# DAGroup-PKU/MHLA

Measured on AMD Instinct MI355X. Metric: MHLA fwd+bwd tokens/sec at (B,N,H,D), higher is better.
Workload: dtype bf16; 1 GPU; block-mix MHLA op fwd+bwd, per GPU B=8 N=4096 H=16 D=64 M=64 S=64 bf16 (BASELINE.json configs[1]); global_batch=8, parallelism=dp1 (batch shards, dW all-reduce only)

## Files before the change

mhla_amd/csrc/capi.hip:

```cpp
#include "capi_common.hpp"
#include "fused.hpp"
#include "fused_tile16.hpp"
#include "smalln.hpp"
#include "smalln_f32.hpp"

using namespace mhla;
using namespace mhla::capi;

namespace mhla {
namespace capi {
extern template int bm_fwd_typed<float, false>(const BmCall&);
extern template int bm_fwd_typed<bf16_t, true>(const BmCall&);
extern template int bm_fwd_typed<bf16_t, false>(const BmCall&);
extern template int bm_fwd_typed<f16_t, false>(const BmCall&);
extern template int bm_bwd_typed<float, false>(const BmCall&);
extern template int bm_bwd_typed<bf16_t, true>(const BmCall&);
extern template int bm_bwd_typed<bf16_t, false>(const BmCall&);
extern template int bm_bwd_typed<f16_t, false>(const BmCall&);
}
}

namespace {

template <int MODE>
// ... 129 lines not shown
}

extern "C" {


int mhla_abi_version(void) { return MHLA_ABI_VERSION; }

#ifndef MHLA_BUILD_FLAGS
#define MHLA_BUILD_FLAGS "unknown"
#endif
const char* mhla_build_flags(void) { return MHLA_BUILD_FLAGS; }

void mhla_prof_enable(int on) {
    std::lock_guard<std::mutex> lk(g_prof_mu);
    g_prof_on = on != 0;
}

int mhla_prof_report(char* buf, size_t cap) {
    std::vector<ProfRec> recs;
    {
        std::lock_guard<std::mutex> lk(g_prof_mu);
        recs.swap(g_prof);
    }
    std::map<std::string, std::pair<long, double>> agg;
    for (auto& r : recs) {
        float ms = 0.f;
        (void)hipEventSynchronize(r.e1);
        (void)hipEventElapsedTime(&ms, r.e0, r.e1);
        auto& a = agg[r.name];
        a.first += 1;
        a.second += ms;
        (void)hipEventDestroy(r.e0);
        (void)hipEventDestroy(r.e1);
    }
    std::string out;
    char line[256];
    for (auto& kv : agg) {
        snprintf(line, sizeof(line), "%s %ld %.6f\n", kv.first.c_str(), kv.second.first, kv.second.second);
        out += line;
    }
    if (!buf || cap == 0) return (int)out.size();
    const size_t n = out.size() < cap - 1 ? out.size() : cap - 1;
    memcpy(buf, out.data(), n);
    buf[n] = 0;
    return (int)n;
}
const char* mhla_last_error(void) { return g_err; }

int mhla_set_option(const char* name, int value) {
    if (name && !strcmp(name, "bwd_two_launches")) return g_two_launches.exchange(value != 0);
    if (name && !strcmp(name, "debug_drop_signal")) return g_drop_signal.exchange(value != 0);
    if (name && !strcmp(name, "fp32_summaries")) return g_no_p24.exchange(value != 0);
    if (name && !strcmp(name, "recut_kernels")) return g_recut.exchange(value != 0);
    return fail(MHLA_EINVAL, "mhla_set_option: unknown option '%s'", name ? name : "(null)");
}

void mhla_debug_set_trace(void* buf) { g_trace = (unsigned long long*)buf; }

int mhla_blockmix_fwd_keeps_state(int B, int H, int M, int S, int D, int dtype, int split, unsigned flags) {
    (void)B; (void)H;
    switch (bm_route(M, S, D, dtype, split != 0, flags)) {
        case BM_SNF: case BM_SN: return 0;
        case BM_FAST: return 1;
        default: return sp_shape_ok(D, flags) ? 1 : 0;
    }
}

size_t mhla_blockmix_fwd_ws_bytes(int B, int H, int M, int S, int D, int dtype, int split, unsigned flags) {
    const size_t gen = bm_carve_for(nullptr, B, H, M, S, D, dtype, flags, true).total_fwd;
    return bm_fast_layout(M, S, D, dtype, split != 0, flags) ? std::max(gen, fast_carve(nullptr, B, H, M, S).total_fwd) : gen;
}
size_t mhla_blockmix_bwd_ws_bytes(int B, int H, int M, int S, int D, int dtype, int split, unsigned flags) {
    return bwd_ws_body_bytes(B, H, M, S, D, dtype, split, flags) + 16;
}

static BmCall bm_call(mhla_view q_num, mhla_view k_num, mhla_view v, mhla_view q_den, mhla_view k_den, const float* W, int ldw, const int32_t* block_index,
                      int B, int H, int M, int S, int D, int dtype, float eps, unsigned flags, void* stream, const float* rcos, const float* rsin, long ldr) {
    BmCall c{};
    c.normalize = q_den.ptr != nullptr;
    c.split = c.normalize && (q_den.ptr != q_num.ptr || k_den.ptr != k_num.ptr);
    c.q_num = q_num; c.k_num = k_num; c.v = v; c.q_den = c.normalize ? q_den : q_num; c.k_den = c.normalize ? k_den : k_num;
    c.W = W; c.ldw = ldw; c.block_index = block_index; c.B = B; c.H = H; c.M = M; c.S = S; c.D = D; c.dtype = dtype; c.eps = eps; c.flags = flags;
    c.st = (hipStream_t)stream; c.rcos = rcos; c.rsin = rsin; c.ldr = ldr;
    return c;
}
static int bm_typed(const BmCall& c, const bool FWD) {
    switch (c.dtype) {
        case MHLA_F32: return FWD ? bm_fwd_typed<float, false>(c) : bm_bwd_typed<float, false>(c);
        case MHLA_BF16:
            if (bm_sum16(c.D, c.dtype, c.flags)) return FWD ? bm_fwd_typed<bf16_t, true>(c) : bm_bwd_typed<bf16_t, true>(c);
            return FWD ? bm_fwd_typed<bf16_t, false>(c) : bm_bwd_typed<bf16_t, false>(c);
        case MHLA_F16: return FWD ? bm_fwd_typed<f16_t, false>(c) : bm_bwd_typed<f16_t, false>(c);
        default: return fail(MHLA_EINVAL, "unknown dtype %d", c.dtype);
    }
}

static fast::SnArgs sn_args(const BmCall& c, void* dwp) {
    fast::SnArgs sa{};
    sa.q = cv(c.q_num); sa.k = cv(c.k_num); sa.v = cv(c.v); sa.idx = c.block_index; sa.W = c.W; sa.ldw = c.ldw;
    sa.H = c.H; sa.M = c.M; sa.D = c.D; sa.eps = c.eps; sa.relu = c.relu(); sa.normalize = c.normalize;
    if (!dwp) { sa.out = cmv(c.out); return sa; }
    sa.o = c.normalize ? cv(c.outv) : cv(c.q_num); sa.dout = cv(c.dout); sa.dq = cmv(c.dq_num); sa.dk = cmv(c.dk_num); sa.dv = cmv(c.dv); sa.dwp = (float*)dwp;
    return sa;
}
static int sn_fwd(const BmCall& c, BmRoute r) {
    const fast::SnArgs sa = sn_args(c, nullptr);
// ... 277 lines not shown
```

mhla_amd/csrc/capi_bm_typed.hpp:

```cpp
#pragma once
#include "capi_common.hpp"
#include "blockmix.hpp"
#include "split.hpp"
#include "split16.hpp"
#include "mixh2.hpp"

namespace mhla {
namespace capi {

static_assert(sp::mixr_te<4, SF_BF16>() == mixr_slice(true) && sp::mixr_te<4, SF_F32>() == mixr_slice(false) && sp::mixr_te<4, SF_P24>() == mixr_slice(false), "bm_plan's resident-mixing rule");
template <int DT> constexpr int sp_state_threads() {
#ifdef MHLA_SP_STATE_4WAVES
    return NTHREADS;
#else
    return DT == 8 ? 512 : NTHREADS;
#endif
}
#ifndef SP_MIXH2_IH
#define SP_MIXH2_IH 2
#endif
#ifndef SP_MIXH2_RT
#define SP_MIXH2_RT 1
#endif

// ... 109 lines not shown
    constexpr bool PACKED = bm_fmt_built<ET, DT, S16, SF_P24>();
    const MixOp o = mix_op(p, c, TRANS);
    const bool wz = c.normalize && p.wz_fused;
    const char* name = p.n_mix[TRANS];
    const MixArgs tiled{o.W, o.ldw, o.in, o.out, o.M, o.E, o.es}, dense{o.W, o.ldw, o.in, o.out, o.M, o.E, TRANS ? 0 : o.es};
    switch (p.mix[TRANS]) {
        case K_MIX:
            return launch(k_mix<TRANS, 0>, dim3((unsigned)((o.E + MIX_TE - 1) / MIX_TE), (o.M + MIX_TI - 1) / MIX_TI, o.BH), dim3(NTHREADS), MIX_SMEM_FLOATS * 4, o.st, name, dense);
        case K_SP_MIX:
            if (p.fmt == PLAIN) return launch(sp::k_sp_mix<TRANS, PLAIN>, dim3((unsigned)((o.E + sp::SPM_TE - 1) / sp::SPM_TE), (o.M + 63) / 64, o.BH), dim3(NTHREADS), sp::sp_mix_smem<PLAIN>(), o.st, name, tiled);
            break;
        case K_SP_MIXR_DMA:
            if constexpr (S16) return sp_mixr_dma<TRANS>(o, wz, name);
            break;
        case K_SP_MIXR:
            if (TRANS == 1 && p.dw_fused) {
                if constexpr (TRANS == 1) {
                    if (p.fmt == SF_P24) { if constexpr (PACKED) return sp_mixr<1, SF_P24, true>(o, p.nw, wz, name, parts); }
                    else if (p.fmt == SF_F32) return sp_mixr<1, SF_F32, true>(o, p.nw, wz, name, parts);
                }
            } else if (p.fmt == SF_P24) { if constexpr (PACKED) return sp_mixr<TRANS, SF_P24, false>(o, p.nw, wz, name); }
            else if (p.fmt == PLAIN) return sp_mixr<TRANS, PLAIN, false>(o, p.nw, wz, name);
            break;
        case K_SP_MIXH: case K_SP_MIXH2:
            if constexpr (PACKED) return sp_mixh<TRANS>(o, p.mix[TRANS], p.nw, TRANS && p.dw_fused, wz, name, parts);
            break;
        default: break;
    }
    return not_built<ET, DT>(name, p.fmt);
}
template <int TRANS>
int launch_wz(const float* W, int ldw, const float* x, float* out, int BH, int M, int S, float eps, hipStream_t st) {
    return launch(k_wz<TRANS>, dim3((S + 63) / 64, (M + 63) / 64, BH), dim3(NTHREADS), 0, st, N_WZ[TRANS], W, ldw, x, out, M, S, eps);
}

template <typename ET, int DT, int TRANS, bool S16>
int bm_state(const BmPlan& p, const BmCall& c, const StateArgs& a) {
    constexpr bool F32 = std::is_same<ET, float>::value;
    constexpr int SNT = sp_state_threads<DT>();
    const dim3 g(c.M, c.B * c.H);
    const char* name = p.n_state[TRANS];
    if (p.state == K_BM_STATE) return launch(k_bm_state<ET, DT, TRANS>, g, dim3(NTHREADS), state_smem_floats<DT>() * 4, c.st, name, a);
    if (p.state == K_S16_STATE) return launch(s16::k_s16_state<TRANS>, dim3((c.M + s16::WPB - 1) / s16::WPB, c.B * c.H), dim3(64 * s16::WPB), s16::state_smem(), c.st, name, a);
    if (p.rope) {
        constexpr sp::StateVar ROPE{.rope = true};
        if (p.fmt == SF_P24) {
            if constexpr (F32 && bm_fmt_built<ET, DT, S16, SF_P24>()) return launch(sp::k_sp_state<ET, DT, TRANS, SNT, SF_P24, ROPE>, g, dim3(SNT), sp::sp_state_smem<DT>(), c.st, name, a);
        } else if (p.fmt == sf_plain<S16>()) {
            if constexpr (F32 || TRANS == 0) return launch(sp::k_sp_state<ET, DT, TRANS, SNT, sf_plain<S16>(), ROPE>, g, dim3(SNT), sp::sp_state_smem<DT>(), c.st, name, a);
        }
        return not_built<ET, DT>(name, p.fmt);
    }
    if constexpr (TRANS == 0 && bm_fmt_built<ET, DT, S16, SF_H16>()) {
        if (p.fmt == SF_H16 && !(c.normalize && c.split) && g_recut.load())
            return launch(sp::k_sp_state<ET, DT, 0, SNT, SF_H16, sp::StateVar{.ts = false}>, g, dim3(SNT), sp::sp_state_smem<DT>(), c.st, name, a);
    }
    return with_fmt<ET, DT, S16>(p.fmt, name, [&]<int FMT>() {
        constexpr int smem = (sf_packed(FMT) && TRANS && sizeof(ET) == 2 && DT <= 4) ? sp::sp_state_rd_smem<DT, sp::sp_payrd<ET, DT, FMT>()>() : sp::sp_state_smem<DT>();
        return launch(sp::k_sp_state<ET, DT, TRANS, SNT, FMT>, g, dim3(SNT), smem, c.st, name, a);
    });
}
template <typename ET, int DT, bool S16>
int bm_state_and_mix(const BmPlan& p, const BmCall& c) {
    const BmWs& w = c.w;
    StateArgs a{};
    a.rcos = c.rcos; a.rsin = c.rsin; a.ldr = c.ldr;
    a.x = cv(c.k_num); a.y = cv(c.v); a.kd = cv(c.k_den); a.qd = cv(c.q_den); a.idx = c.block_index;
    a.out = w.kv; a.ksum = w.ksum; a.zo = w.z; a.es = w.es;
    a.H = c.H; a.M = c.M; a.S = c.S; a.D = c.D; a.eps = c.eps; a.relu = c.relu(); a.normalize = c.normalize; a.split = c.split;
    RC((bm_state<ET, DT, 0, S16>(p, c, a)));
    RC((bm_mix<ET, DT, 0, S16>(p, c)));
    if (p.wz_kernel) RC(launch_wz<0>(c.W, c.ldw, w.z, w.ninv, c.B * c.H, c.M, c.S, c.eps, c.st));
    return MHLA_OK;
}

template <typename ET, int DT, bool S16, typename TO = ET, bool EPI = false>
int sp_out(const BmPlan& p, const BmCall& c, const OutArgs& o, const char* name) {
    const dim3 g(c.M, c.B * c.H), blk(sp::SP_OUT_T);
    if constexpr (!EPI && bm_fmt_built<ET, DT, S16, SF_H16>() && DT <= 4) {
        if (p.fmt == SF_H16 && bm_one_tile(c.S))
            return launch(sp::k_sp_out<ET, DT, TO, SF_H16, sp::OutVar{.one = true}>, g, blk, sp::sp_out_smem<DT, SF_H16>(), c.st, name, o);
    }
    return with_fmt<ET, DT, S16>(p.fmt, name, [&]<int FMT>() {
        return launch(sp::k_sp_out<ET, DT, TO, FMT, sp::OutVar{.epi = EPI}>, g, blk, sp::sp_out_smem<DT, FMT>(), c.st, name, o);
    });
}
inline OutArgs out_args(const BmCall& c) {
    OutArgs o{};
    o.rcos = c.rcos; o.rsin = c.rsin; o.ldr = c.ldr;
    o.q = cv(c.q_num); o.idx = c.block_index; o.W = c.W; o.ldw = c.ldw; o.g = c.w.g; o.ninv = c.w.ninv;
    o.H = c.H; o.M = c.M; o.S = c.S; o.D = c.D; o.eps = c.eps; o.es = c.w.es; o.relu = c.relu(); o.normalize = c.normalize;
    return o;
}
template <typename ET, int DT, bool S16>
int bm_out(const BmPlan& p, const BmCall& c, OutArgs& o, const char* name) {
    if (p.out == K_BM_OUT) return launch(k_bm_out<ET, DT>, dim3(c.M, c.B * c.H), dim3(NTHREADS), out_smem_floats<DT>() * 4, c.st, name, o);
    if (p.out == K_S16_OUT) return launch(s16::k_s16_out<0>, dim3((c.M + s16::WPB - 1) / s16::WPB, c.B * c.H), dim3(64 * s16::WPB), s16::out_smem(), c.st, name, o);
    if (!c.epi) return sp_out<ET, DT, S16>(p, c, o, name);
    if constexpr (std::is_same<ET, float>::value) {
        o.nw = c.nw; o.neps = c.neps; o.gate = cv(c.gate);
        if (c.out_dtype == MHLA_BF16) return sp_out<float, DT, S16, bf16_t, true>(p, c, o, name);
        if (c.out_dtype == MHLA_F16) return sp_out<float, DT, S16, f16_t, true>(p, c, o, name);
        return sp_out<float, DT, S16, float, true>(p, c, o, name);
    }
    return not_built<ET, DT>(name, p.fmt);
}

inline int sp_dwr_splits(int BH, long E) {
    int ns = (256 + BH - 1) / BH;
    if (ns > DW_MAX_SPLIT) ns = DW_MAX_SPLIT;
    while (ns > 1 && E / ns < 256) --ns;
// ... 149 lines not shown
```

mhla_amd/csrc/capi_common.hpp:

```cpp
#pragma once
#include "../../include/mhla_hip.h"

#include <algorithm>
#include <atomic>
#include <cstdarg>
#include <cstdio>
#include <cstdlib>
#include <cstring>
#include <map>
#include <mutex>
#include <string>
#include <vector>

#include "common.hpp"

namespace mhla {
namespace capi {


inline thread_local char g_err[512] = "";

inline int fail(int code, const char* fmt, ...) {
    va_list ap;
    va_start(ap, fmt);
// ... 9 lines not shown
inline std::atomic<bool> g_prof_on{false};
inline std::vector<ProfRec> g_prof;

template <typename K>
int launch(K kernel, dim3 grid, dim3 block, size_t smem, hipStream_t stream, const char* name, auto... args) {
    if (smem > 48 * 1024) {
        static std::mutex mu;
        static std::map<std::pair<const void*, int>, size_t> done;
        int dev = 0;
        (void)hipGetDevice(&dev);
        const std::pair<const void*, int> key(reinterpret_cast<const void*>(kernel), dev);
        std::lock_guard<std::mutex> lk(mu);
        auto it = done.find(key);
        if (it == done.end() || it->second < smem) {
            hipError_t e = hipFuncSetAttribute(key.first, hipFuncAttributeMaxDynamicSharedMemorySize, (int)smem);
            if (e != hipSuccess) return fail(MHLA_ELAUNCH, "%s: hipFuncSetAttribute(%zu B LDS): %s", name, smem, hipGetErrorString(e));
            done[key] = smem;
        }
    }
    ProfRec rec{name, nullptr, nullptr};
    const bool prof = g_prof_on;
    if (prof) {
        (void)hipEventCreate(&rec.e0);
        (void)hipEventCreate(&rec.e1);
        (void)hipEventRecord(rec.e0, stream);
    }
    hipLaunchKernelGGL(kernel, grid, block, smem, stream, args...);
    if (prof) {
        (void)hipEventRecord(rec.e1, stream);
        std::lock_guard<std::mutex> lk(g_prof_mu);
        g_prof.push_back(rec);
    }
    hipError_t e = hipGetLastError();
    if (e != hipSuccess) return fail(MHLA_ELAUNCH, "%s: launch failed: %s", name, hipGetErrorString(e));
    return MHLA_OK;
}

inline std::atomic<unsigned long long*> g_trace{nullptr};

#ifndef SP_MIXH2_MIN_SLICES
#define SP_MIXH2_MIN_SLICES 8
#endif
#ifndef SP_MIXH2_TE
#define SP_MIXH2_TE 64
#endif
inline std::atomic<int> g_recut{[] { const char* e = getenv("MHLA_RECUT"); const char* f = getenv("MHLA_WAN_FLAT"); return ((e && e[0] == '0') || (f && f[0] == '0')) ? 0 : 1; }()};
inline bool sp_mixh2_applies(int M, long E, long BH, long S = 0) {
    if (M <= 128 || M > 256 || !g_recut.load()) return false;
    if (BH * M * (E / 2 + 288) * 4 >= (1L << 31) || BH * M * S * 4 >= (1L << 31)) return false;
    const long total = BH * ((E + SP_MIXH2_TE - 1) / SP_MIXH2_TE), wgs = std::min<long>(total, 256);
    return wgs > 0 && (total + wgs - 1) / wgs >= SP_MIXH2_MIN_SLICES;
}
inline bool bm_one_tile(int S) { return S <= 64 && g_recut.load(); }
inline std::atomic<int> g_no_p24{[] { const char* e = getenv("MHLA_FP32_SUMMARIES"); return (e && e[0] == '1') ? 1 : 0; }()};

inline View cv(const mhla_view& v) { return View{v.ptr, (long)v.sb, (long)v.sn, (long)v.sh}; }
inline MView cmv(const mhla_mview& v) { return MView{v.ptr, (long)v.sb, (long)v.sn, (long)v.sh}; }

inline int check_view(const char* name, const void* ptr, int64_t sb, int64_t sn, int64_t sh, int dtype) {
    if (!ptr) return fail(MHLA_EINVAL, "%s: null pointer", name);
    const int esz = dtype == MHLA_F32 ? 4 : 2;
    if (((uintptr_t)ptr) % (4 * esz) != 0) return fail(MHLA_EINVAL, "%s: pointer not %d-byte aligned", name, 4 * esz);
    if ((sb | sn | sh) & 3) return fail(MHLA_EINVAL, "%s: strides (%lld, %lld, %lld) must be multiples of 4 elements", name,
                                        (long long)sb, (long long)sn, (long long)sh);
    return MHLA_OK;
}
#define CHECK_VIEW(v) do { int rc_ = check_view(#v, (v).ptr, (v).sb, (v).sn, (v).sh, dtype); if (rc_) return rc_; } while (0)
#define RC(x) do { int rc_ = (x); if (rc_) return rc_; } while (0)

constexpr int DW_MAX_SPLIT = 16;
inline int dw_splits(long wgs, long E) {
    long ns = (1024 + wgs - 1) / wgs;
    if (ns > DW_MAX_SPLIT) ns = DW_MAX_SPLIT;
    while (ns > 1 && E / ns < 256) --ns;
    return (int)(ns < 1 ? 1 : ns);
}

inline int dt_for(int D) { return D <= 32 ? 2 : D <= 64 ? 4 : D <= 80 ? 5 : D <= 96 ? 6 : D <= 128 ? 8 : 0; }

#define DISPATCH_T(dtype, ...)                                                   \
    switch (dtype) {                                                             \
        case MHLA_F32: { using ET = float; __VA_ARGS__; break; }                  \
        case MHLA_BF16: { using ET = bf16_t; __VA_ARGS__; break; }                \
        case MHLA_F16: { using ET = f16_t; __VA_ARGS__; break; }                  \
        default: return fail(MHLA_EINVAL, "unknown dtype %d", dtype);            \
    }
#define DISPATCH_DT(dt, ...)                                                     \
    switch (dt) {                                                                \
        case 2: { constexpr int DT = 2; __VA_ARGS__; break; }                    \
        case 4: { constexpr int DT = 4; __VA_ARGS__; break; }                    \
        case 5: { constexpr int DT = 5; __VA_ARGS__; break; }                    \
        case 6: { constexpr int DT = 6; __VA_ARGS__; break; }                    \
        case 8: { constexpr int DT = 8; __VA_ARGS__; break; }                    \
        default: return fail(MHLA_ENOTSUP, "head dim tile %d not supported", dt);\
    }

struct BmWs {
    float *kv, *g, *z, *ksum, *ninv, *dg, *dkv, *dn, *dz, *dks, *dwp;
    unsigned short* olo;
    size_t total_fwd, total_bwd;
    long es;
    int fmt;
};
inline long bm_row_elems(int D, int fmt, bool padded) {
    const long E = (long)D * D;
    switch (fmt) {
// ... 216 lines not shown
```

mhla_amd/csrc/split.hpp:

```cpp
#pragma once
#include <type_traits>

#include "blockmix.hpp"
#include "fused.hpp"

namespace mhla {
namespace sp {

using fast::bf16x8;
using fast::mfma_bf16;
using fast::tr_read8;
using fast::s16x4;
using fast::s16x8;
using fast::u16;

__device__ __forceinline__ bf16x8 row_read8(const u16* tile, int ld, int c0, int k0, int lane) {
    return *reinterpret_cast<const bf16x8*>(tile + (c0 + (lane & 15)) * ld + k0 + (lane >> 4) * 8);
}

template <typename T>
__device__ __forceinline__ void ld8(const T* p, f32x4& a, f32x4& b) {
    a = Io<T>::ld4(p);
    b = Io<T>::ld4(p + 4);
}
// ... 197 lines not shown
#pragma unroll
    for (int u = 0; u < PASSES; ++u) {
        const int r = min(r0 + RPP * u, D - 1), c = min(cg, D - 8);
        x16[u] = gld<uint4>(rowp + 2 * (r * D + c));
    }
#pragma unroll
    for (int u = 0; u < PASSES; ++u) {
        const int r = r0 + RPP * u;
        if (r < KP && cg < KP) *reinterpret_cast<uint4*>(G + mat_row<mat_new<DT>()>(r) * LD + cg) = (r < D && cg < D) ? x16[u] : make_uint4(0, 0, 0, 0);
    }
    return hm;
}

template <int DT, int NT>
struct MatStage {
    static constexpr int PASSES = (Geo<DT>::KST * 32 + NT / Geo<DT>::CGS - 1) / (NT / Geo<DT>::CGS);
    uint4 x16[PASSES];
    uint2 xl[PASSES];
};
template <int DT, int NT>
__device__ __forceinline__ void stage_mat_issue(MatStage<DT, NT>& g, const float* __restrict__ base, long elem_off, int D, int tid, bool real = true) {
    constexpr int CGS = Geo<DT>::CGS, RPP = NT / CGS;
    const int r0 = tid / CGS, cg = (tid % CGS) * 8;
    const char* rowp = reinterpret_cast<const char*>(base + elem_off);
#pragma unroll
    for (int u = 0; u < MatStage<DT, NT>::PASSES; ++u) {
        const int r = min(r0 + RPP * u, D - 1), c = min(cg, D - 8), e = real ? r * D + c : 0;
        g.x16[u] = gld<uint4>(rowp + 2 * e);
        g.xl[u] = gld<uint2>(rowp + 2 * D * D + e);
    }
}
template <int DT, int NT>
__device__ __forceinline__ void stage_mat_commit(u16* __restrict__ Gh, u16* __restrict__ Gl, const MatStage<DT, NT>& g, int D, int tid) {
    constexpr int LD = mat_ld<DT>(), CGS = Geo<DT>::CGS, RPP = NT / CGS, KP = Geo<DT>::KST * 32;
    const int r0 = tid / CGS, cg = (tid % CGS) * 8;
#pragma unroll
    for (int u = 0; u < MatStage<DT, NT>::PASSES; ++u) {
        const int r = r0 + RPP * u, off = mat_row<mat_new<DT>()>(r) * LD + cg;
        const bool in = r < D && cg < D;
        const uint4 hi = in ? g.x16[u] : make_uint4(0, 0, 0, 0);
        const uint2 lo = in ? g.xl[u] : make_uint2(0, 0);
        if (r < KP && cg < KP) {
            *reinterpret_cast<uint4*>(Gh + off) = hi;
            *reinterpret_cast<uint4*>(Gl + off) = p24_lo8(hi, lo);
        }
    }
}

template <int DT>
__host__ __device__ constexpr int sp_state_smem() {
    static_assert(Geo<DT>::RPP * Geo<DT>::DW * 4 <= 4 * 32 * Geo<DT>::LD * 2, "column-sum partials must fit in the tiles");
    return 4 * 32 * Geo<DT>::LD * 2 + Geo<DT>::DW * 4;
}

template <int DT, bool ONEP = false> __host__ __device__ constexpr int sp_state_rd_smem() {
    return 4 * 32 * (ONEP ? Geo<DT>::LD : Geo<DT>::LDR) * 2 + Geo<DT>::DW * 4 + (ONEP ? 1 : 2) * Geo<DT>::KST * 32 * mat_ld<DT>() * 2 + 2 * 32 * 4;
}
template <typename T, int DT, int FMT>
__host__ __device__ constexpr bool sp_payrd() { return sp_payop<T, DT, FMT>() && std::is_same<T, bf16_t>::value; }
static_assert(!SP_PAYLOAD_OPERANDS || 5 * sp_state_rd_smem<4, true>() <= 160 * 1024, "five k_sp_state<1> (row dots from G) workgroups per CU at D = 64");

struct StateVar { bool rope = false, pro = false, ts = true; };
template <typename T, int DT, int MODE, int NT, int FMT, StateVar V = StateVar{}>
__global__ __launch_bounds__(NT, NT == 512 ? 4 : (V.rope ? 2 : 3)) void k_sp_state(const StateArgs a) {
    constexpr bool ROPE = V.rope, PRO = V.pro, TS = V.ts;
    static_assert(TS || MODE == 0, "the backward's third tensor is a property of its arithmetic (RD), not of the call");
    static_assert(!PRO || (MODE == 0 && FMT != SF_BF16), "the prologue on load serves the forward's summary kernel on fp32-grade summaries");
    constexpr bool RD = MODE == 1 && sf_packed(FMT) && sizeof(T) == 2 && DT <= 4 && !ROPE;
    constexpr bool THIRD = TS && !RD;
    constexpr bool PAYRD = RD && sp_payrd<T, DT, FMT>();
    constexpr bool TN = !RD || PAYRD;
    constexpr int DW = Geo<DT>::DW, LD = TN ? Geo<DT>::LD : Geo<DT>::LDR, CGS = Geo<DT>::CGS, RPP = NT / CGS, IT = 32 / RPP, NWV = NT / 64,
                  RT = (DT + NWV - 1) / NWV, TILE = 32 * LD;
    static_assert(IT >= 1 && RPP * IT == 32, "a 32-row chunk must be whole staging passes");
    static_assert(RPP * DW * 4 <= 4 * 32 * LD * 2, "column-sum partials must fit in the tiles");
    constexpr bool LO = !std::is_same<T, bf16_t>::value || PRO;
    constexpr bool LOY = !std::is_same<T, bf16_t>::value || (MODE == 1 && sf_has_lo(FMT));
    constexpr int GLD = mat_ld<DT>(), GT = Geo<DT>::KST * 32 * GLD;
    extern __shared__ __attribute__((aligned(16))) unsigned char smem_raw[];
    u16* Kh = reinterpret_cast<u16*>(smem_raw);
    u16* Kl = Kh + TILE;
    u16* Vh = Kl + TILE;
    u16* Vl = Vh + TILE;
    float* cs = reinterpret_cast<float*>(smem_raw);
    float* vecd = reinterpret_cast<float*>(Vl + TILE);
    u16* Gh = reinterpret_cast<u16*>(vecd + DW);
    u16* Gl = Gh + GT;
    float* rdp = reinterpret_cast<float*>(Gh + (PAYRD ? 1 : 2) * GT);
    const int tid = threadIdx.x, wave = __builtin_amdgcn_readfirstlane(tid >> 6), lane = tid & 63, nl = lane & 15, kg = lane >> 4;
    const int blk = blockIdx.x, bh = blockIdx.y, b = bh / a.H, h = bh - b * a.H, S = a.S, D = a.D;
    const long p0 = (long)blk * S;
    const T* kb = (const T*)a.x.ptr + b * a.x.sb + h * a.x.sh;
    const T* vb = (const T*)a.y.ptr + b * a.y.sb + h * a.y.sh;
    const View& third = MODE == 0 ? a.kd : a.o;
    const T* kdb = (const T*)third.ptr + b * third.sb + h * third.sh;
    const bool den = THIRD && a.normalize && ((MODE == 1 && !RD) || (MODE == 0 && a.split));
    const int r0 = tid / CGS, cg = (tid % CGS) * 8;
    const float* ninvb = a.ninv + ((long)bh * a.M + blk) * S;

    typename Raw4<T>::type kr[IT][2], vr[IT][2], dr[THIRD ? IT : 1][2];
    f32x4 kx[IT][2], vx[IT][2], dx[THIRD ? IT : 1][2], rc[ROPE ? IT : 1], rs[ROPE ? IT : 1];
    float nv[IT];
    float prr[PRO ? IT : 1];
    f32x4 pw[PRO ? 2 : 1];
    constexpr bool rope = ROPE;
    int crow = 0;
    int nraw[IT], npos[IT];
    auto lookup = [&](int c0) __attribute__((always_inline)) {
#pragma unroll
        for (int it = 0; it < IT; ++it) {
            const long p = p0 + min(c0 + r0 + RPP * it, S - 1);
            nraw[it] = gld<int>(a.idx ? (const void*)(a.idx + p) : a.x.ptr);
            npos[it] = (int)p;
        }
    };
    lookup(0);
    const int cgc = min(cg, D - 8);
    if constexpr (PRO) {
        pw[0] = pw[1] = f32x4{1.f, 1.f, 1.f, 1.f};
        if (a.pro_wk) {
            pw[0] = *reinterpret_cast<const f32x4*>(a.pro_wk + h * D + cgc);
            pw[1] = *reinterpret_cast<const f32x4*>(a.pro_wk + h * D + cgc + 4);
        }
    }
    const T* kdq = den ? kdb : kb;
    const long kdsn = den ? third.sn : a.x.sn;
    const float* nvp = (MODE == 1 && a.normalize) ? ninvb : reinterpret_cast<const float*>(a.x.ptr);
    constexpr bool OLO = MODE == 1 && sf_has_lo(FMT) && sizeof(T) == 2 && !RD;
    const bool olo_on = OLO && a.normalize && a.olo != nullptr;
    const u16* olop = olo_on ? a.olo + ((long)bh * a.M * S + p0) * D + cgc : reinterpret_cast<const u16*>(a.x.ptr);
    uint4 ox[OLO ? IT : 1];
    auto fetch = [&](int c0) __attribute__((always_inline)) {
        crow = c0;
#pragma unroll
        for (int it = 0; it < IT; ++it) {
            const int rcl = min(c0 + r0 + RPP * it, S - 1);
            const long row = a.idx ? nraw[it] : npos[it];
            kr[it][0] = gld<typename Raw4<T>::type>(kb + row * a.x.sn + cgc);
            kr[it][1] = gld<typename Raw4<T>::type>(kb + row * a.x.sn + cgc + 4);
            vr[it][0] = gld<typename Raw4<T>::type>(vb + row * a.y.sn + cgc);
            vr[it][1] = gld<typename Raw4<T>::type>(vb + row * a.y.sn + cgc + 4);
            if constexpr (THIRD) {
                dr[it][0] = gld<typename Raw4<T>::type>(kdq + row * kdsn + cgc);
                dr[it][1] = gld<typename Raw4<T>::type>(kdq + row * kdsn + cgc + 4);
            }
            nv[it] = gld<float>(nvp + ((MODE == 1 && a.normalize) ? rcl : 0));
            if constexpr (PRO) prr[it] = gld<float>(a.pro_rk ? a.pro_rk + b * a.pro_n + row : reinterpret_cast<const float*>(a.x.ptr));
            if constexpr (OLO) ox[it] = gld<uint4>(olop + (olo_on ? (long)rcl * D : 0));
            if constexpr (rope) {
                rc[it] = *reinterpret_cast<const f32x4*>(a.rcos + row * a.ldr + cgc / 2);
                rs[it] = *reinterpret_cast<const f32x4*>(a.rsin + row * a.ldr + cgc / 2);
            }
        }
        lookup(c0 + 32);
    };
    auto settle = [&]() __attribute__((always_inline)) {
#pragma unroll
        for (int it = 0; it < IT; ++it) {
            const bool valid = crow + r0 + RPP * it < S && cg < D;
            const f32x4 z4 = {0.f, 0.f, 0.f, 0.f};
#pragma unroll
            for (int hf = 0; hf < 2; ++hf) {
                kx[it][hf] = raw4_to_f32(T{}, kr[it][hf]);
                vx[it][hf] = raw4_to_f32(T{}, vr[it][hf]);
                if constexpr (THIRD) dx[it][hf] = raw4_to_f32(T{}, dr[it][hf]);
            }
            if constexpr (PRO) {
                const float r = a.pro_rk ? prr[it] : 1.f;
                kx[it][0] = (kx[it][0] * r) * pw[0];
// ... 36 lines not shown
                if constexpr (THIRD) {
                    float d = 0.f;
#pragma unroll
                    for (int i = 0; i < 4; ++i) d += vx[it][0][i] * dx[it][0][i] + vx[it][1][i] * dx[it][1][i];
#pragma unroll
                    for (int o = CGS / 2; o > 0; o >>= 1) d += __shfl_xor(d, o, 64);
                    const int r = crow + r0 + RPP * it;
                    if (r < S && (tid % CGS) == 0) a.dn[((long)bh * a.M + blk) * S + r] = -d * nv[it];
                } else {
                    nvc[it] = nv[it];
                    crowc = crow;
                    if constexpr (PAYRD) {
                        float mx = 0.f;
#pragma unroll
                        for (int i = 0; i < 4; ++i) mx = fmaxf(mx, fmaxf(fabsf(vx[it][0][i]), fabsf(vx[it][1][i])));
                        const float u = tok16_scale<1, CGS>(mx);
                        *reinterpret_cast<uint4*>(Kl + off) = h16_pack8(vx[it][0], vx[it][1], u);
                        nvc[it] = ((gm * nv[it]) * h16_inv(u)) * nv[it];
                    }
                }
                vx[it][0] *= nv[it];
                vx[it][1] *= nv[it];
            }
            if constexpr (rope) {
                f32x4 r0 = kx[it][0], r1 = kx[it][1];
                rope8(r0, r1, rc[it], rs[it]);
                split8(r0, r1, hi, lo);
            } else {
                split8(kx[it][0], kx[it][1], hi, lo);
            }
            *reinterpret_cast<uint4*>(Kh + off) = hi;
            if (LO) *reinterpret_cast<uint4*>(Kl + off) = lo;
            split8(vx[it][0], vx[it][1], hi, lo);
            *reinterpret_cast<uint4*>(Vh + off) = hi;
            if (LOY) *reinterpret_cast<uint4*>(Vl + off) = lo;
            if (MODE == 0) {
                const f32x4* s = kx[it];
                if constexpr (THIRD) s = den ? dx[it] : kx[it];
#pragma unroll
                for (int i = 0; i < 4; ++i) {
                    ksp[i] += s[0][i];
                    ksp[4 + i] += s[1][i];
                }
            }
        }
    };

    f32x4 acc[RT][DT];
#pragma unroll
    for (int i = 0; i < RT; ++i)
#pragma unroll
        for (int j = 0; j < DT; ++j) acc[i][j] = f32x4{0.f, 0.f, 0.f, 0.f};

    fetch(0);
    if constexpr (RD) {
        if (a.normalize) {
            if constexpr (PAYRD) gm = stage_mat_payload<DT, NT>(Gh, a.g, ((long)bh * a.M + blk) * a.es, D, tid);
            else stage_mat_split<DT, FMT, NT>(Gh, Gl, a.g, ((long)bh * a.M + blk) * a.es, D, tid);
        }
    }
    auto chunk = [&]<bool PF>(std::bool_constant<PF>, int c0) __attribute__((always_inline)) {
        commit();
        __syncthreads();
        if constexpr (PF) fetch(c0 + 32);
        if constexpr (RD) {
            if (a.normalize) {
                constexpr int KSTG = Geo<DT>::KST, CTH = (DT + 1) / 2;
                const int tt = wave & 1, hf = wave >> 1;
                bf16x8 bh_[KSTG], bl_[KSTG];
#pragma unroll
                for (int ks = 0; ks < KSTG; ++ks) {
                    bh_[ks] = mat_row_read8<TN>(PAYRD ? Kl : Vh, LD, tt * 16, ks * 32, lane);
                    if constexpr (!PAYRD) bl_[ks] = mat_row_read8<TN>(Vl, LD, tt * 16, ks * 32, lane);
                }
                float dot = 0.f;
#pragma unroll
                for (int c = 0; c < CTH; ++c) {
                    const int ct = hf * CTH + c;
                    if (ct < DT) {
                        f32x4 t4 = {0.f, 0.f, 0.f, 0.f};
#pragma unroll
                        for (int ks = 0; ks < KSTG; ++ks) {
                            const bf16x8 gh = mat_row_read8<mat_new<DT>()>(Gh, GLD, ct * 16, ks * 32, lane);
                            if constexpr (PAYRD) {
                                t4 = fast::mfma_f16(fast::as_f16x8(gh), fast::as_f16x8(bh_[ks]), t4);
                            } else {
                                const bf16x8 gl = mat_row_read8<mat_new<DT>()>(Gl, GLD, ct * 16, ks * 32, lane);
                                t4 = mfma_bf16(gh, bh_[ks], t4);
                                t4 = mfma_bf16(gl, bh_[ks], t4);
                                t4 = mfma_bf16(gh, bl_[ks], t4);
                            }
                        }
                        const uint2 qr = *reinterpret_cast<const uint2*>(Kh + (tt * 16 + mat_row<TN>(nl)) * LD + ct * 16 + kg * 4);
                        f32x4 q4 = {__uint_as_float(qr.x << 16), __uint_as_float(qr.x & 0xffff0000u), __uint_as_float(qr.y << 16), __uint_as_float(qr.y & 0xffff0000u)};
                        if (LO) {
                            const uint2 ql = *reinterpret_cast<const uint2*>(Kl + (tt * 16 + mat_row<TN>(nl)) * LD + ct * 16 + kg * 4);
                            q4 += f32x4{__uint_as_float(ql.x << 16), __uint_as_float(ql.x & 0xffff0000u), __uint_as_float(ql.y << 16), __uint_as_float(ql.y & 0xffff0000u)};
                        }
                        dot += t4[0] * q4[0] + t4[1] * q4[1] + t4[2] * q4[2] + t4[3] * q4[3];
                    }
                }
                dot += __shfl_xor(dot, 16, 64);
                dot += __shfl_xor(dot, 32, 64);
                if (kg == 0) rdp[hf * 32 + tt * 16 + nl] = dot;
            }
        }
        bf16x8 ah[RT], al[RT];
#pragma unroll
        for (int rt = 0; rt < RT; ++rt) {
            const int c0 = min(wave * RT + rt, DW / 16 - 1) * 16;
            ah[rt] = mat_tr_read8<TN>(Kh, LD, 0, c0, lane);
            if (LO) al[rt] = mat_tr_read8<TN>(Kl, LD, 0, c0, lane);
        }
#pragma unroll
        for (int ct = 0; ct < DT; ++ct) {
            const bf16x8 bh_ = mat_tr_read8<TN>(Vh, LD, 0, ct * 16, lane);
#pragma unroll
            for (int rt = 0; rt < RT; ++rt) acc[rt][ct] = mfma_bf16(ah[rt], bh_, acc[rt][ct]);
            if (LOY) {
                const bf16x8 bl_ = mat_tr_read8<TN>(Vl, LD, 0, ct * 16, lane);
#pragma unroll
                for (int rt = 0; rt < RT; ++rt) acc[rt][ct] = mfma_bf16(ah[rt], bl_, acc[rt][ct]);
            }
            if (LO) {
#pragma unroll
                for (int rt = 0; rt < RT; ++rt) acc[rt][ct] = mfma_bf16(al[rt], bh_, acc[rt][ct]);
            }
        }
        __syncthreads();
        if constexpr (RD) {
            if (a.normalize && (tid % CGS) == 0) {
#pragma unroll
                for (int it = 0; it < IT; ++it) {
                    const int lr = r0 + RPP * it, r = crowc + lr;
                    if (r < S) a.dn[((long)bh * a.M + blk) * S + r] = -(rdp[lr] + rdp[32 + lr]) * nvc[it];
                }
            }
        }
    };
    int c0 = 0;
    for (; c0 + 32 < S; c0 += 32) chunk(std::true_type{}, c0);
    chunk(std::false_type{}, c0);

    float* ob = a.out + ((long)bh * a.M + blk) * a.es;
    constexpr int CW = (DW > 64 && NWV == 8) ? 64 : DW, LDO = CW + 4, PPRO = CW / 4;
    static_assert(NWV * 16 * LDO * 4 <= 4 * 32 * LD * 2, "the staging tiles of all waves must fit in the operand tiles");
    const bool staged = sf_has_lo(FMT) && (sf_packed(FMT) || ((D & 3) == 0 && (a.es & 3) == 0));
    float hinv = 0.f;
    if constexpr (FMT == SF_H16) {
        float mx = 0.f;
#pragma unroll
        for (int rt = 0; rt < RT; ++rt)
#pragma unroll
            for (int ct = 0; ct < DT; ++ct)
#pragma unroll
                for (int r = 0; r < 4; ++r) mx = fmaxf(mx, fabsf(acc[rt][ct][r]));
#pragma unroll
        for (int o = 32; o > 0; o >>= 1) mx = fmaxf(mx, __shfl_xor(mx, o, 64));
        if (lane == 0) vecd[wave] = mx;
        __syncthreads();
#pragma unroll
        for (int w = 0; w < NWV; ++w) mx = fmaxf(mx, vecd[w]);
        const float hm = h16_mult_from_max(mx);
        hinv = h16_inv(hm);
        if (tid == 0) gst<float>(reinterpret_cast<char*>(ob) + 2 * D * D, hm);
    }
    if (staged) {
        float* Os = reinterpret_cast<float*>(smem_raw) + wave * 16 * LDO;
#pragma unroll
        for (int rt = 0; rt < RT; ++rt) {
            const int tile = wave * RT + rt;
            if (tile * 16 < D) {
#pragma unroll
                for (int c0 = 0; c0 < DW; c0 += CW) {
#pragma unroll
                    for (int ct = c0 / 16; ct < (c0 + CW) / 16; ++ct)
                        if (ct < DT)
#pragma unroll
                            for (int r = 0; r < 4; ++r) Os[(kg * 4 + r) * LDO + ct * 16 - c0 + nl] = acc[rt][ct][r];
                    __builtin_amdgcn_wave_barrier();
                    if constexpr (sf_packed(FMT)) {
#pragma unroll
                        for (int p = 0; p < CW / 32; ++p) {
                            const int v = lane + 64 * p, row = v / (CW / 8), c8 = v % (CW / 8);
                            const int grow = tile * 16 + row, gcol = c0 + c8 * 8;
                            if (grow < D && gcol < D) {
                                const float* src = Os + row * LDO + c8 * 8;
                                const int e = grow * D + gcol;
                                if constexpr (FMT == SF_H16) {
                                    gst<uint4>(reinterpret_cast<char*>(ob) + 2 * e, h16_pack8(*reinterpret_cast<const f32x4*>(src), *reinterpret_cast<const f32x4*>(src + 4), hinv));
                                } else {
                                uint4 hi;
                                uint2 lo;
                                p24_pack8(*reinterpret_cast<const f32x4*>(src), *reinterpret_cast<const f32x4*>(src + 4), hi, lo);
                                gst<uint4>(reinterpret_cast<char*>(ob) + 2 * e, hi);
                                gst<uint2>(reinterpret_cast<char*>(ob) + 2 * D * D + e, lo);
                                }
                            }
                        }
                    } else {
#pragma unroll
                    for (int p = 0; p < CW / 16; ++p) {
                        const int v = lane + 64 * p, row = v / PPRO, c4 = v % PPRO;
                        const int grow = tile * 16 + row, gcol = c0 + c4 * 4;
                        if (grow < D && gcol < D) gst<f32x4>(ob + (long)grow * D + gcol, *reinterpret_cast<const f32x4*>(Os + row * LDO + c4 * 4));
                    }
                    }
                    __builtin_amdgcn_wave_barrier();
                }
            }
        }
        if (MODE == 0 && a.normalize) __syncthreads();
    } else {
#pragma unroll
    for (int rt = 0; rt < RT; ++rt)
#pragma unroll
        for (int ct = 0; ct < DT; ++ct)
#pragma unroll
            for (int r = 0; r < 4; ++r) {
                const int row = (wave * RT + rt) * 16 + kg * 4 + r, col = ct * 16 + nl;
                if (row < D && col < D) {
                    if (FMT == SF_BF16) reinterpret_cast<u16*>(a.out)[((long)bh * a.M + blk) * a.es + (long)row * D + col] = cvt_bf16(acc[rt][ct][r]);
                    else                 ob[(long)row * D + col] = acc[rt][ct][r];
                }
            }
    }

    if (MODE == 0 && a.normalize) {
#pragma unroll
        for (int i = 0; i < 8; ++i) cs[r0 * DW + cg + i] = ksp[i];
        __syncthreads();
        if (tid < DW) {
            float s = 0.f;
#pragma unroll 4
            for (int r = 0; r < RPP; ++r) s += cs[r * DW + tid];
            vecd[tid] = s;
            if (tid < D) a.ksum[((long)bh * a.M + blk) * D + tid] = s;
        }
        __syncthreads();
        const T* qb = (const T*)a.qd.ptr + b * a.qd.sb + h * a.qd.sh;
        float kv8[8];
#pragma unroll
        for (int i = 0; i < 8; ++i) kv8[i] = vecd[cg + i];
        f32x4 qw[PRO ? 2 : 1];
        if constexpr (PRO) {
            qw[0] = qw[1] = f32x4{1.f, 1.f, 1.f, 1.f};
            if (a.pro_wq && cg < D) {
                qw[0] = *reinterpret_cast<const f32x4*>(a.pro_wq + h * D + cg);
                qw[1] = *reinterpret_cast<const f32x4*>(a.pro_wq + h * D + cg + 4);
            }
        }
        constexpr int ZB = 4;
        for (int rb = 0; rb < S; rb += RPP * ZB) {
            f32x4 x0[ZB], x1[ZB];
            int rw[ZB];
            if (a.idx) {
#pragma unroll
                for (int u = 0; u < ZB; ++u) rw[u] = gld<int>(a.idx + p0 + min(rb + u * RPP + r0, S - 1));
            } else {
#pragma unroll
                for (int u = 0; u < ZB; ++u) rw[u] = (int)p0 + min(rb + u * RPP + r0, S - 1);
            }
#pragma unroll
            for (int u = 0; u < ZB; ++u) {
                const int r = rb + u * RPP + r0;
                x0[u] = x1[u] = f32x4{0.f, 0.f, 0.f, 0.f};
                if (r < S && cg < D) ld8(qb + (long)rw[u] * a.qd.sn + cg, x0[u], x1[u]);
            }
#pragma unroll
            for (int u = 0; u < ZB; ++u) {
                const int r = rb + u * RPP + r0;
                float d = 0.f;
                if (r < S && cg < D) {
                    if constexpr (PRO) {
                        const float rq = a.pro_rq ? a.pro_rq[b * a.pro_n + rw[u]] : 1.f;
                        x0[u] = (x0[u] * rq) * qw[0];
                        x1[u] = (x1[u] * rq) * qw[1];
                    }
                    if (a.relu) relu8(x0[u], x1[u], a.eps);
#pragma unroll
                    for (int i = 0; i < 4; ++i) d += x0[u][i] * kv8[i] + x1[u][i] * kv8[4 + i];
                }
#pragma unroll
                for (int o = CGS / 2; o > 0; o >>= 1) d += __shfl_xor(d, o, 64);
                if (r < S && (tid % CGS) == 0) a.zo[((long)bh * a.M + blk) * S + r] = d;
            }
        }
    }
}

constexpr int SPM_TE = 128, SPM_LD = SPM_TE + 8, SPM_TILE = 32 * SPM_LD;
constexpr int SP_MIX_SMEM = 4 * SPM_TILE * 2;
static_assert(64 * (SPM_TE + 4) * 4 <= SP_MIX_SMEM, "output staging must fit in the input tiles");
constexpr int SP_MIX_SMEM16 = 2 * SPM_TILE * 2;
static_assert(64 * SPM_LD * 2 <= SP_MIX_SMEM16, "bf16 output staging must fit in the input tiles");
template <int FMT> constexpr int sp_mix_smem() { return FMT == SF_BF16 ? SP_MIX_SMEM16 : SP_MIX_SMEM; }
// ... 1760 lines not shown
```

Before: 101.7 million tokens/s.

## Add one-fetch state kernel variant that issues all row loads up front for S<=64

Adds a `.one` variant of the summary-state kernel for h16 summaries of 16-bit tensors when the block fits one tile (S<=64). Every global load is issued at kernel start: both 32-row halves of K and V, the normalizer q rows, and the G matrix for the backward. This replaces the per-chunk prefetch pipeline. The forward variant also uses a slimmer shared-memory layout with fewer operand tiles, raises launch bounds to allow more workgroups per CU, and computes the z outputs from registers before returning early. The trade-off is higher register pressure and more code paths, in exchange for more latency hiding and occupancy.

```diff
diff --git a/mhla_amd/csrc/capi.hip b/mhla_amd/csrc/capi.hip
--- a/mhla_amd/csrc/capi.hip
+++ b/mhla_amd/csrc/capi.hip
@@ -205,6 +205,7 @@
     if (name && !strcmp(name, "debug_drop_signal")) return g_drop_signal.exchange(value != 0);
     if (name && !strcmp(name, "fp32_summaries")) return g_no_p24.exchange(value != 0);
     if (name && !strcmp(name, "recut_kernels")) return g_recut.exchange(value != 0);
+    if (name && !strcmp(name, "state_one_fetch")) return g_state_one.exchange(value != 0);
     return fail(MHLA_EINVAL, "mhla_set_option: unknown option '%s'", name ? name : "(null)");
 }
 
diff --git a/mhla_amd/csrc/capi_bm_typed.hpp b/mhla_amd/csrc/capi_bm_typed.hpp
--- a/mhla_amd/csrc/capi_bm_typed.hpp
+++ b/mhla_amd/csrc/capi_bm_typed.hpp
@@ -185,11 +185,21 @@
         return not_built<ET, DT>(name, p.fmt);
     }
     if constexpr (TRANS == 0 && bm_fmt_built<ET, DT, S16, SF_H16>()) {
-        if (p.fmt == SF_H16 && !(c.normalize && c.split) && g_recut.load())
+        if (p.fmt == SF_H16 && !(c.normalize && c.split) && g_recut.load()) {
+            if constexpr (DT <= 4) {
+                constexpr int smem1 = std::is_same<ET, bf16_t>::value ? sp::sp_state_slim_smem<DT>() : sp::sp_state_smem<DT>();
+                if (bm_state_one_fetch(c.S))
+                    return launch(sp::k_sp_state<ET, DT, 0, SNT, SF_H16, sp::StateVar{.ts = false, .one = true}>, g, dim3(SNT), smem1, c.st, name, a);
+            }
             return launch(sp::k_sp_state<ET, DT, 0, SNT, SF_H16, sp::StateVar{.ts = false}>, g, dim3(SNT), sp::sp_state_smem<DT>(), c.st, name, a);
+        }
     }
     return with_fmt<ET, DT, S16>(p.fmt, name, [&]<int FMT>() {
         constexpr int smem = (sf_packed(FMT) && TRANS && sizeof(ET) == 2 && DT <= 4) ? sp::sp_state_rd_smem<DT, sp::sp_payrd<ET, DT, FMT>()>() : sp::sp_state_smem<DT>();
+        if constexpr (FMT == SF_H16 && TRANS == 1 && sizeof(ET) == 2 && DT <= 4) {
+            if (bm_state_one_fetch(c.S))
+                return launch(sp::k_sp_state<ET, DT, 1, SNT, SF_H16, sp::StateVar{.one = true}>, g, dim3(SNT), smem, c.st, name, a);
+        }
         return launch(sp::k_sp_state<ET, DT, TRANS, SNT, FMT>, g, dim3(SNT), smem, c.st, name, a);
     });
 }
diff --git a/mhla_amd/csrc/capi_common.hpp b/mhla_amd/csrc/capi_common.hpp
--- a/mhla_amd/csrc/capi_common.hpp
+++ b/mhla_amd/csrc/capi_common.hpp
@@ -85,6 +85,8 @@
     return wgs > 0 && (total + wgs - 1) / wgs >= SP_MIXH2_MIN_SLICES;
 }
 inline bool bm_one_tile(int S) { return S <= 64 && g_recut.load(); }
+inline std::atomic<int> g_state_one{[] { const char* e = getenv("MHLA_STATE_ONE_FETCH"); return (e && e[0] == '0') ? 0 : 1; }()};
+inline bool bm_state_one_fetch(int S) { return bm_one_tile(S) && g_state_one.load(); }
 inline std::atomic<int> g_no_p24{[] { const char* e = getenv("MHLA_FP32_SUMMARIES"); return (e && e[0] == '1') ? 1 : 0; }()};
 
 inline View cv(const mhla_view& v) { return View{v.ptr, (long)v.sb, (long)v.sn, (long)v.sh}; }
diff --git a/mhla_amd/csrc/split.hpp b/mhla_amd/csrc/split.hpp
--- a/mhla_amd/csrc/split.hpp
+++ b/mhla_amd/csrc/split.hpp
@@ -273,6 +273,12 @@
     static_assert(Geo<DT>::RPP * Geo<DT>::DW * 4 <= 4 * 32 * Geo<DT>::LD * 2, "column-sum partials must fit in the tiles");
     return 4 * 32 * Geo<DT>::LD * 2 + Geo<DT>::DW * 4;
 }
+template <int DT>
+__host__ __device__ constexpr int sp_state_slim_body() {
+    constexpr int tiles = 2 * 32 * Geo<DT>::LD * 2, stage = 4 * 16 * (Geo<DT>::DW + 4) * 4, cs = Geo<DT>::RPP * Geo<DT>::DW * 4;
+    return tiles > stage ? (tiles > cs ? tiles : cs) : (stage > cs ? stage : cs);
+}
+template <int DT> __host__ __device__ constexpr int sp_state_slim_smem() { return sp_state_slim_body<DT>() + Geo<DT>::DW * 4; }
 
 template <int DT, bool ONEP = false> __host__ __device__ constexpr int sp_state_rd_smem() {
     return 4 * 32 * (ONEP ? Geo<DT>::LD : Geo<DT>::LDR) * 2 + Geo<DT>::DW * 4 + (ONEP ? 1 : 2) * Geo<DT>::KST * 32 * mat_ld<DT>() * 2 + 2 * 32 * 4;
@@ -281,10 +287,12 @@
 __host__ __device__ constexpr bool sp_payrd() { return sp_payop<T, DT, FMT>() && std::is_same<T, bf16_t>::value; }
 static_assert(!SP_PAYLOAD_OPERANDS || 5 * sp_state_rd_smem<4, true>() <= 160 * 1024, "five k_sp_state<1> (row dots from G) workgroups per CU at D = 64");
 
-struct StateVar { bool rope = false, pro = false, ts = true; };
+struct StateVar { bool rope = false, pro = false, ts = true, one = false; };
 template <typename T, int DT, int MODE, int NT, int FMT, StateVar V = StateVar{}>
-__global__ __launch_bounds__(NT, NT == 512 ? 4 : (V.rope ? 2 : 3)) void k_sp_state(const StateArgs a) {
-    constexpr bool ROPE = V.rope, PRO = V.pro, TS = V.ts;
+__global__ __launch_bounds__(NT, NT == 512 ? 4 : (V.rope ? 2 : ((V.one && MODE == 0 && std::is_same<T, bf16_t>::value) ? 8 : 3))) void k_sp_state(const StateArgs a) {
+    constexpr bool ROPE = V.rope, PRO = V.pro, TS = V.ts, ONE = V.one;
+    static_assert(!ONE || (FMT == SF_H16 && sizeof(T) == 2 && DT <= 4 && NT == 256 && !ROPE && !PRO), "the one-fetch form: h16 summaries of 16-bit tensors, D <= 64");
+    static_assert(!ONE || MODE == 1 || !TS, "the forward's one-fetch form has no third row stream");
     static_assert(TS || MODE == 0, "the backward's third tensor is a property of its arithmetic (RD), not of the call");
     static_assert(!PRO || (MODE == 0 && FMT != SF_BF16), "the prologue on load serves the forward's summary kernel on fp32-grade summaries");
     constexpr bool RD = MODE == 1 && sf_packed(FMT) && sizeof(T) == 2 && DT <= 4 && !ROPE;
@@ -301,10 +309,11 @@
     extern __shared__ __attribute__((aligned(16))) unsigned char smem_raw[];
     u16* Kh = reinterpret_cast<u16*>(smem_raw);
     u16* Kl = Kh + TILE;
-    u16* Vh = Kl + TILE;
+    constexpr bool SLIM = ONE && MODE == 0 && !LO && !LOY;
+    u16* Vh = SLIM ? Kl : Kl + TILE;
     u16* Vl = Vh + TILE;
     float* cs = reinterpret_cast<float*>(smem_raw);
-    float* vecd = reinterpret_cast<float*>(Vl + TILE);
+    float* vecd = SLIM ? reinterpret_cast<float*>(smem_raw + sp_state_slim_body<DT>()) : reinterpret_cast<float*>(Vl + TILE);
     u16* Gh = reinterpret_cast<u16*>(vecd + DW);
     u16* Gl = Gh + GT;
     float* rdp = reinterpret_cast<float*>(Gh + (PAYRD ? 1 : 2) * GT);
@@ -335,7 +344,7 @@
             npos[it] = (int)p;
         }
     };
-    lookup(0);
+    if constexpr (!ONE) lookup(0);
     const int cgc = min(cg, D - 8);
     if constexpr (PRO) {
         pw[0] = pw[1] = f32x4{1.f, 1.f, 1.f, 1.f};
@@ -478,12 +487,75 @@
 #pragma unroll
         for (int j = 0; j < DT; ++j) acc[i][j] = f32x4{0.f, 0.f, 0.f, 0.f};
 
+    constexpr int GP = (Geo<DT>::KST * 32 + RPP - 1) / RPP;
+    typename Raw4<T>::type kr2[2], vr2[2], qz[2][2];
+    float nv2 = 1.f;
+    uint4 gx[GP];
+    if constexpr (ONE) {
+        static_assert(IT == 1 && RD == (MODE == 1) && !THIRD, "one row per thread and half; the backward takes its row dots from G_i");
+        long row[2];
+        if (a.idx) {
+            row[0] = gld<int>(a.idx + p0 + min(r0, S - 1));
+            row[1] = gld<int>(a.idx + p0 + min(r0 + 32, S - 1));
+        } else {
+            row[0] = (int)p0 + min(r0, S - 1);
+            row[1] = (int)p0 + min(r0 + 32, S - 1);
+        }
+        const bool nrm = MODE == 1 && a.normalize;
+        kr[0][0] = gld<typename Raw4<T>::type>(kb + row[0] * a.x.sn + cgc);
+        kr[0][1] = gld<typename Raw4<T>::type>(kb + row[0] * a.x.sn + cgc + 4);
+        vr[0][0] = gld<typename Raw4<T>::type>(vb + row[0] * a.y.sn + cgc);
+        vr[0][1] = gld<typename Raw4<T>::type>(vb + row[0] * a.y.sn + cgc + 4);
+        nv[0] = 1.f;
+        if constexpr (MODE == 1) nv[0] = gld<float>(nvp + (nrm ? min(r0, S - 1) : 0));
+        if constexpr (RD) {
+            const char* gp = nrm ? reinterpret_cast<const char*>(a.g + ((long)bh * a.M + blk) * a.es) : reinterpret_cast<const char*>(a.x.ptr);
+            gm = gld<float>(gp + (nrm ? 2 * D * D : 0));
+#pragma unroll
+            for (int u = 0; u < GP; ++u) gx[u] = gld<uint4>(gp + (nrm ? 2 * (min(r0 + RPP * u, D - 1) * D + cgc) : 0));
+        }
+        kr2[0] = gld<typename Raw4<T>::type>(kb + row[1] * a.x.sn + cgc);
+        kr2[1] = gld<typename Raw4<T>::type>(kb + row[1] * a.x.sn + cgc + 4);
+        vr2[0] = gld<typename Raw4<T>::type>(vb + row[1] * a.y.sn + cgc);
+        vr2[1] = gld<typename Raw4<T>::type>(vb + row[1] * a.y.sn + cgc + 4);
+        if constexpr (MODE == 1) nv2 = gld<float>(nvp + (nrm ? min(r0 + 32, S - 1) : 0));
+        if constexpr (MODE == 0) {
+            const T* qb = a.normalize ? (const T*)a.qd.ptr + b * a.qd.sb + h * a.qd.sh : kb;
+            const long qsn = a.normalize ? a.qd.sn : a.x.sn;
+#pragma unroll
+            for (int hf = 0; hf < 2; ++hf) {
+                qz[hf][0] = gld<typename Raw4<T>::type>(qb + row[hf] * qsn + cgc);
+                qz[hf][1] = gld<typename Raw4<T>::type>(qb + row[hf] * qsn + cgc + 4);
+            }
+        }
+        if constexpr (RD) {
+            gm = a.normalize ? gm : 1.f;
+#pragma unroll
+            for (int u = 0; u < GP; ++u) {
+                const int r = r0 + RPP * u, off = mat_row<mat_new<DT>()>(r) * GLD + cg;
+                const bool in = r < D && cg < D;
+                uint4 x16 = gx[u];
+                x16.x = in ? x16.x : 0u; x16.y = in ? x16.y : 0u; x16.z = in ? x16.z : 0u; x16.w = in ? x16.w : 0u;
+                if (r < Geo<DT>::KST * 32 && cg < Geo<DT>::KST * 32) {
+                    if constexpr (PAYRD) {
+                        *reinterpret_cast<uint4*>(Gh + off) = x16;
+                    } else {
+                        uint4 hi, lo;
+                        h16_split8(x16, gm, hi, lo);
+                        *reinterpret_cast<uint4*>(Gh + off) = hi;
+                        *reinterpret_cast<uint4*>(Gl + off) = lo;
+                    }
+                }
+            }
+        }
+    } else {
     fetch(0);
     if constexpr (RD) {
         if (a.normalize) {
             if constexpr (PAYRD) gm = stage_mat_payload<DT, NT>(Gh, a.g, ((long)bh * a.M + blk) * a.es, D, tid);
             else stage_mat_split<DT, FMT, NT>(Gh, Gl, a.g, ((long)bh * a.M + blk) * a.es, D, tid);
         }
+    }
     }
     auto chunk = [&]<bool PF>(std::bool_constant<PF>, int c0) __attribute__((always_inline)) {
         commit();
@@ -564,13 +636,26 @@
             }
         }
     };
+    if constexpr (ONE) {
+        chunk(std::false_type{}, 0);
+        if (S > 32) {
+            kr[0][0] = kr2[0]; kr[0][1] = kr2[1];
+            vr[0][0] = vr2[0]; vr[0][1] = vr2[1];
+            nv[0] = nv2;
+            crow = 32;
+            chunk(std::false_type{}, 32);
+        }
+    } else {
     int c0 = 0;
     for (; c0 + 32 < S; c0 += 32) chunk(std::true_type{}, c0);
     chunk(std::false_type{}, c0);
+    }
 
     float* ob = a.out + ((long)bh * a.M + blk) * a.es;
     constexpr int CW = (DW > 64 && NWV == 8) ? 64 : DW, LDO = CW + 4, PPRO = CW / 4;
     static_assert(NWV * 16 * LDO * 4 <= 4 * 32 * LD * 2, "the staging tiles of all waves must fit in the operand tiles");
+    static_assert(!SLIM || (NWV * 16 * LDO * 4 <= sp_state_slim_body<DT>() && RPP * DW * 4 <= sp_state_slim_body<DT>() && 2 * TILE * 2 <= sp_state_slim_body<DT>()),
+                  "the slim body holds the two tiles, the staging tiles and the column-sum partials");
     const bool staged = sf_has_lo(FMT) && (sf_packed(FMT) || ((D & 3) == 0 && (a.es & 3) == 0));
     float hinv = 0.f;
     if constexpr (FMT == SF_H16) {
@@ -668,6 +753,23 @@
         float kv8[8];
 #pragma unroll
         for (int i = 0; i < 8; ++i) kv8[i] = vecd[cg + i];
+        if constexpr (ONE) {
+#pragma unroll
+            for (int hf = 0; hf < 2; ++hf) {
+                const int r = hf * 32 + r0;
+                f32x4 x0 = raw4_to_f32(T{}, qz[hf][0]), x1 = raw4_to_f32(T{}, qz[hf][1]);
+                float d = 0.f;
+                if (r < S && cg < D) {
+                    if (a.relu) relu8(x0, x1, a.eps);
+#pragma unroll
+                    for (int i = 0; i < 4; ++i) d += x0[i] * kv8[i] + x1[i] * kv8[4 + i];
+                }
+#pragma unroll
+                for (int o = CGS / 2; o > 0; o >>= 1) d += __shfl_xor(d, o, 64);
+                if (r < S && (tid % CGS) == 0) a.zo[((long)bh * a.M + blk) * S + r] = d;
+            }
+            return;
+        }
         f32x4 qw[PRO ? 2 : 1];
         if constexpr (PRO) {
             qw[0] = qw[1] = f32x4{1.f, 1.f, 1.f, 1.f};
```

Result: faster. 103.0 million tokens/s (median of 6 runs) (+1.3%).
